# submission2019/cnn-quantization

Measured on NVIDIA H100. Metric: resnet50_w4a4_images_per_s, higher is better.
Workload: dtype f32

## Files before the change

cnn-quantization_b200/csrc/fq_bulk.cuh:

```cuda
#pragma once
#include <cuda_runtime.h>
#include <stdint.h>

#include "fq_device.cuh"

namespace fqb {

constexpr int kConsumers = kThreads;
constexpr int kBulkThreads = kConsumers + 32;
constexpr int kConsumerWarps = kConsumers / 32;
#ifndef FQB_STAGE_VEC
#define FQB_STAGE_VEC 4
#endif
#ifndef FQB_STAGES
#define FQB_STAGES 6
#endif
#ifndef FQB_BULK_CTAS
#define FQB_BULK_CTAS 1
#endif
constexpr int kBulkCtasPerSm = FQB_BULK_CTAS;
constexpr int kStageVec = FQB_STAGE_VEC;
constexpr int kStages = FQB_STAGES;
constexpr unsigned kStageBytes = kStageVec * kConsumers * 16u;
#ifndef FQB_BULK_SPLIT
#define FQB_BULK_SPLIT 1
#endif
constexpr unsigned kBulkSplit = FQB_BULK_SPLIT;

__device__ __forceinline__ void consumer_sync() { cta_sync(); }

__device__ __forceinline__ unsigned smem_u32(const void* p) { return static_cast<unsigned>(__cvta_generic_to_shared(p)); }
__device__ __forceinline__ void mbar_init(unsigned bar, unsigned count) {
  asm volatile("mbarrier.init.shared::cta.b64 [%0], %1;" ::"r"(bar), "r"(count) : "memory");
}
__device__ __forceinline__ void mbar_fence_init() { asm volatile("fence.mbarrier_init.release.cluster;" ::: "memory"); }
__device__ __forceinline__ void mbar_arrive(unsigned bar) {
  asm volatile("{ .reg .b64 st; mbarrier.arrive.shared::cta.b64 st, [%0]; }" ::"r"(bar) : "memory");
}
__device__ __forceinline__ void mbar_arrive_expect_tx(unsigned bar, unsigned bytes) {
  asm volatile("{ .reg .b64 st; mbarrier.arrive.expect_tx.shared::cta.b64 st, [%0], %1; }" ::"r"(bar), "r"(bytes) : "memory");
}
__device__ __forceinline__ bool mbar_try_wait(unsigned bar, unsigned parity) {
  unsigned ok;
  asm volatile(
      "{ .reg .pred p; mbarrier.try_wait.parity.shared::cta.b64 p, [%1], %2; selp.u32 %0, 1, 0, p; }"
      : "=r"(ok)
      : "r"(bar), "r"(parity)
      : "memory");
  return ok != 0;
}
__device__ __forceinline__ void mbar_wait(unsigned bar, unsigned parity) {
  while (!mbar_try_wait(bar, parity)) {
  }
}
__device__ __forceinline__ void bulk_load_one(unsigned dst_smem, const void* src, unsigned bytes, unsigned bar) {
  asm volatile("cp.async.bulk.shared::cluster.global.mbarrier::complete_tx::bytes [%0], [%1], %2, [%3];" ::"r"(dst_smem),
               "l"(src), "r"(bytes), "r"(bar)
               : "memory");
}
__device__ __forceinline__ void bulk_load(unsigned dst_smem, const void* src, unsigned bytes, unsigned bar) {
  if (kBulkSplit == 1u) {
    bulk_load_one(dst_smem, src, bytes, bar);
    return;
  }
  constexpr unsigned piece = kStageBytes / kBulkSplit;
  for (unsigned off = 0; off < bytes; off += piece)
    bulk_load_one(dst_smem + off, static_cast<const unsigned char*>(src) + off, min(piece, bytes - off), bar);
}

struct FlatGeo {
  unsigned total_v;
  unsigned stride;
  unsigned stage_v;
  unsigned n_stages;
  unsigned unit_stages;
  unsigned units;
  unsigned channels;
  unsigned cv;
};

struct StageMeta {
  unsigned start;
  unsigned count;
  unsigned tag;
  unsigned pad;
};

struct BulkRing {
  alignas(8) unsigned long long full[kStages];
  alignas(8) unsigned long long empty[kStages];
  StageMeta meta[kStages];
  unsigned nstages;
};

struct RingPos {
  unsigned slot, parity, n;
  __device__ __forceinline__ void init(unsigned nstages = kStages) {
    slot = 0;
    parity = 0;
    n = nstages;
  }
  __device__ __forceinline__ void next() {
    if (++slot == n) {
      slot = 0;
      parity ^= 1u;
    }
  }
};

__device__ __forceinline__ void ring_init(BulkRing& r, unsigned nstages = kStages) {
  if (threadIdx.x == 0) {
    r.nstages = nstages;
#pragma unroll
    for (int s = 0; s < kStages; ++s) {
      mbar_init(smem_u32(&r.full[s]), 1u);
      mbar_init(smem_u32(&r.empty[s]), kConsumerWarps);
    }
    mbar_fence_init();
  }
  __syncthreads();
}

struct TicketPlan {
  unsigned nstatic;
  unsigned first, step;
  unsigned dyn_base;
};

constexpr unsigned kPairOffset = kStageBytes / 2u;

__device__ __forceinline__ FlatGeo half_geo(const FlatGeo& g) {
  FlatGeo h = g;
  h.stage_v = (kStageVec / 2u) * g.stride;
  h.n_stages = (g.total_v + h.stage_v - 1u) / h.stage_v;
  h.unit_stages = 2u * g.unit_stages;
  return h;
}

template <bool REV, bool PAIR = false>
__device__ __forceinline__ void produce_phase(const FlatGeo& g, const float4* src, unsigned* counter, const TicketPlan tp,
                                              BulkRing& r, unsigned char* stage_base, RingPos& pos,
                                              const float4* src2 = nullptr) {
  const unsigned total = g.units;
  unsigned k = 0;
  auto fetch = [&]() -> unsigned {
    unsigned long long t;
    if (k < tp.nstatic)
      t = tp.first + static_cast<unsigned long long>(k) * tp.step;
    else
      t = static_cast<unsigned long long>(tp.dyn_base) + atomicAdd(counter, 1u);
    ++k;
    return t < total ? static_cast<unsigned>(t) : 0xffffffffu;
  };
  unsigned cur = fetch();
  unsigned nxt = (cur != 0xffffffffu) ? fetch() : 0xffffffffu;
  while (cur != 0xffffffffu) {
    const unsigned nxt2 = (nxt != 0xffffffffu) ? fetch() : 0xffffffffu;
    const unsigned u = REV ? total - 1u - cur : cur;
    const unsigned g0 = u * g.unit_stages;
    const unsigned g1 = min(g0 + g.unit_stages, g.n_stages);
    for (unsigned i = g0; i < g1; ++i) {
      const unsigned st = REV ? g1 - 1u - (i - g0) : i;
      const unsigned start = st * g.stage_v;
      const unsigned count = min(g.stage_v, g.total_v - start);
      mbar_wait(smem_u32(&r.empty[pos.slot]), pos.parity ^ 1u);
      r.meta[pos.slot].start = start;
      r.meta[pos.slot].count = count;
      r.meta[pos.slot].tag = 0u;
      const unsigned bar = smem_u32(&r.full[pos.slot]);
      mbar_arrive_expect_tx(bar, PAIR ? count * 32u : count * 16u);
      bulk_load(smem_u32(stage_base + pos.slot * kStageBytes), src + start, count * 16u, bar);
      if (PAIR) bulk_load(smem_u32(stage_base + pos.slot * kStageBytes + kPairOffset), src2 + start, count * 16u, bar);
      pos.next();
    }
    cur = nxt;
    nxt = nxt2;
  }
  mbar_wait(smem_u32(&r.empty[pos.slot]), pos.parity ^ 1u);
  r.meta[pos.slot].start = 0u;
  r.meta[pos.slot].count = 0u;
  mbar_arrive(smem_u32(&r.full[pos.slot]));
  pos.next();
}

struct RowsGeo {
  unsigned rows, row_v;
  unsigned stages_per_row;
  unsigned units_per_row;
};

__device__ __forceinline__ RowsGeo half_rows(const FlatGeo& h, const RowsGeo& rg) {
  RowsGeo r = rg;
  r.stages_per_row = (rg.row_v + h.stage_v - 1u) / h.stage_v;
  r.units_per_row = (r.stages_per_row + h.unit_stages - 1u) / h.unit_stages;
  return r;
}

template <bool REV, bool PAIR = false>
__device__ __forceinline__ void produce_rows_phase(const FlatGeo& g, const RowsGeo& rg, const float4* src, unsigned* counter,
                                                   const TicketPlan tp, BulkRing& r, unsigned char* stage_base, RingPos& pos,
                                                   const float4* src2 = nullptr) {
  const unsigned total = g.units;
  unsigned k = 0;
  auto fetch = [&]() -> unsigned {
    unsigned long long t;
    if (k < tp.nstatic)
      t = tp.first + static_cast<unsigned long long>(k) * tp.step;
    else
      t = static_cast<unsigned long long>(tp.dyn_base) + atomicAdd(counter, 1u);
    ++k;
    return t < total ? static_cast<unsigned>(t) : 0xffffffffu;
  };
  unsigned cur = fetch();
  unsigned nxt = (cur != 0xffffffffu) ? fetch() : 0xffffffffu;
  while (cur != 0xffffffffu) {
    const unsigned nxt2 = (nxt != 0xffffffffu) ? fetch() : 0xffffffffu;
    const unsigned u = REV ? total - 1u - cur : cur;
    const unsigned row = u / rg.units_per_row;
    const unsigned part = u - row * rg.units_per_row;
    const unsigned s0 = part * g.unit_stages;
    const unsigned s1 = min(s0 + g.unit_stages, rg.stages_per_row);
    for (unsigned i = s0; i < s1; ++i) {
      const unsigned st = REV ? s1 - 1u - (i - s0) : i;
      const unsigned off = st * g.stage_v;
      const unsigned start = row * rg.row_v + off;
      const unsigned count = min(g.stage_v, rg.row_v - off);
      mbar_wait(smem_u32(&r.empty[pos.slot]), pos.parity ^ 1u);
      r.meta[pos.slot].start = start;
      r.meta[pos.slot].count = count;
      r.meta[pos.slot].tag = row | (i + 1u == s1 ? 0x80000000u : 0u);
      const unsigned bar = smem_u32(&r.full[pos.slot]);
      mbar_arrive_expect_tx(bar, PAIR ? count * 32u : count * 16u);
      bulk_load(smem_u32(stage_base + pos.slot * kStageBytes), src + start, count * 16u, bar);
      if (PAIR) bulk_load(smem_u32(stage_base + pos.slot * kStageBytes + kPairOffset), src2 + start, count * 16u, bar);
      pos.next();
    }
    cur = nxt;
    nxt = nxt2;
  }
  mbar_wait(smem_u32(&r.empty[pos.slot]), pos.parity ^ 1u);
  r.meta[pos.slot].start = 0u;
  r.meta[pos.slot].count = 0u;
  r.meta[pos.slot].tag = 0u;
  mbar_arrive(smem_u32(&r.full[pos.slot]));
  pos.next();
}

struct PoolGeo {
  unsigned h, w;
  unsigned wt;
  unsigned tiles_per_row;
  unsigned row_pairs;
  unsigned tiles;
  unsigned unit_tiles, units;
  unsigned ow;
  unsigned kind;
};

constexpr unsigned kPoolTop = 1u, kPoolLeft = 2u;

__device__ __forceinline__ void produce_pool3_phase(const FlatGeo& g, const PoolGeo& pg, const float4* src, unsigned* counter,
                                                    const TicketPlan tp, BulkRing& r, unsigned char* stage_base, RingPos& pos) {
  const unsigned total = pg.units;
  unsigned k = 0;
  auto fetch = [&]() -> unsigned {
    unsigned long long t;
    if (k < tp.nstatic)
      t = tp.first + static_cast<unsigned long long>(k) * tp.step;
    else
      t = static_cast<unsigned long long>(tp.dyn_base) + atomicAdd(counter, 1u);
    ++k;
    return t < total ? static_cast<unsigned>(t) : 0xffffffffu;
  };
  const unsigned row_v = pg.w * g.cv;
  const unsigned region_v = (2u * pg.wt + 1u) * g.cv;
  const unsigned per_img = pg.row_pairs * pg.tiles_per_row;
  unsigned cur = fetch();
  unsigned nxt = (cur != 0xffffffffu) ? fetch() : 0xffffffffu;
  while (cur != 0xffffffffu) {
    const unsigned nxt2 = (nxt != 0xffffffffu) ? fetch() : 0xffffffffu;
    const unsigned t0 = cur * pg.unit_tiles;
    const unsigned t1 = min(t0 + pg.unit_tiles, pg.tiles);
    for (unsigned tile = t0; tile < t1; ++tile) {
      const unsigned n = tile / per_img;
      const unsigned rem = tile - n * per_img;
      const unsigned oh = rem / pg.tiles_per_row;
      const unsigned wi = rem - oh * pg.tiles_per_row;
      const bool top = oh > 0u, left = wi > 0u;
      const unsigned skip = left ? 0u : g.cv;
      const unsigned count = region_v - skip;
      const unsigned mid = (n * pg.h + 2u * oh) * row_v + (2u * wi * pg.wt) * g.cv - (left ? g.cv : 0u);
      const unsigned o = ((n * pg.row_pairs + oh) * pg.ow + wi * pg.wt) * g.cv;
      mbar_wait(smem_u32(&r.empty[pos.slot]), pos.parity ^ 1u);
      r.meta[pos.slot].start = o;
      r.meta[pos.slot].count = count;
      r.meta[pos.slot].tag = (top ? kPoolTop : 0u) | (left ? kPoolLeft : 0u);
      const unsigned bar = smem_u32(&r.full[pos.slot]);
      mbar_arrive_expect_tx(bar, count * 16u * (top ? 3u : 2u));
      const unsigned dst = smem_u32(stage_base + pos.slot * kStageBytes) + skip * 16u;
      if (top) bulk_load(dst, src + mid - row_v, count * 16u, bar);
      bulk_load(dst + region_v * 16u, src + mid, count * 16u, bar);
      bulk_load(dst + 2u * region_v * 16u, src + mid + row_v, count * 16u, bar);
      pos.next();
    }
    cur = nxt;
    nxt = nxt2;
  }
  mbar_wait(smem_u32(&r.empty[pos.slot]), pos.parity ^ 1u);
  r.meta[pos.slot].start = 0u;
  r.meta[pos.slot].count = 0u;
  r.meta[pos.slot].tag = 0u;
  mbar_arrive(smem_u32(&r.full[pos.slot]));
  pos.next();
}

template <typename Acc>
__device__ __forceinline__ void consume_pool3_phase(const FlatGeo& g, const PoolGeo& pg, BulkRing& r, const unsigned char* stage_base,
                                                    RingPos& pos, Acc& acc) {
  const unsigned t = threadIdx.x;
  const bool lane0 = (t & 31u) == 0u;
  const bool mine = t < pg.wt * g.cv;
  const unsigned j = t / g.cv, col = t - j * g.cv;
  const unsigned region = (2u * pg.wt + 1u) * g.cv * 16u;
  const unsigned my = smem_u32(stage_base) + ((2u * j) * g.cv + col) * 16u;
  const unsigned nxt = g.cv * 16u;
  for (;;) {
    mbar_wait(smem_u32(&r.full[pos.slot]), pos.parity);
    const StageMeta m = r.meta[pos.slot];
    if (m.count != 0u && mine) {
      const unsigned addr = my + pos.slot * kStageBytes;
      const bool first = (j != 0u) || (m.tag & kPoolLeft);
      acc.pool_begin();
#pragma unroll
      for (int dy = 0; dy < 3; ++dy) {
        if (dy == 0 && !(m.tag & kPoolTop)) continue;
        const unsigned row = addr + dy * region;
        float4 v;
        if (first) {
          lds_vec(row, v);
          acc.pool_tap(v);
        }
        lds_vec(row + nxt, v);
        acc.pool_tap(v);
        lds_vec(row + 2u * nxt, v);
        acc.pool_tap(v);
      }
      acc.pool_end(m.start + t);
    }
    __syncwarp();
    if (lane0) mbar_arrive(smem_u32(&r.empty[pos.slot]));
    pos.next();
    if (m.count == 0u) break;
  }
}

__device__ __forceinline__ void produce_pool_phase(const FlatGeo& g, const PoolGeo& pg, const float4* src, unsigned* counter,
                                                   const TicketPlan tp, BulkRing& r, unsigned char* stage_base, RingPos& pos) {
  const unsigned total = pg.units;
  unsigned k = 0;
  auto fetch = [&]() -> unsigned {
    unsigned long long t;
    if (k < tp.nstatic)
      t = tp.first + static_cast<unsigned long long>(k) * tp.step;
    else
      t = static_cast<unsigned long long>(tp.dyn_base) + atomicAdd(counter, 1u);
    ++k;
    return t < total ? static_cast<unsigned>(t) : 0xffffffffu;
  };
  const unsigned row_v = pg.w * g.cv;
  const unsigned count = pg.wt * g.cv;
  const unsigned per_img = pg.row_pairs * pg.tiles_per_row;
  unsigned cur = fetch();
  unsigned nxt = (cur != 0xffffffffu) ? fetch() : 0xffffffffu;
  while (cur != 0xffffffffu) {
    const unsigned nxt2 = (nxt != 0xffffffffu) ? fetch() : 0xffffffffu;
    const unsigned t0 = cur * pg.unit_tiles;
    const unsigned t1 = min(t0 + pg.unit_tiles, pg.tiles);
    for (unsigned tile = t0; tile < t1; ++tile) {
      const unsigned n = tile / per_img;
      const unsigned rem = tile - n * per_img;
      const unsigned hp = rem / pg.tiles_per_row;
      const unsigned wi = rem - hp * pg.tiles_per_row;
      const unsigned a = (n * pg.h + 2u * hp) * row_v + wi * count;
      const unsigned o = ((n * pg.row_pairs + hp) * pg.ow + wi * (pg.wt / 2u)) * g.cv;
      mbar_wait(smem_u32(&r.empty[pos.slot]), pos.parity ^ 1u);
      r.meta[pos.slot].start = o;
      r.meta[pos.slot].count = count;
      r.meta[pos.slot].tag = 0u;
      const unsigned bar = smem_u32(&r.full[pos.slot]);
      mbar_arrive_expect_tx(bar, count * 32u);
      bulk_load(smem_u32(stage_base + pos.slot * kStageBytes), src + a, count * 16u, bar);
      bulk_load(smem_u32(stage_base + pos.slot * kStageBytes + kPairOffset), src + a + row_v, count * 16u, bar);
      pos.next();
    }
    cur = nxt;
    nxt = nxt2;
  }
  mbar_wait(smem_u32(&r.empty[pos.slot]), pos.parity ^ 1u);
  r.meta[pos.slot].start = 0u;
  r.meta[pos.slot].count = 0u;
  r.meta[pos.slot].tag = 0u;
  mbar_arrive(smem_u32(&r.full[pos.slot]));
  pos.next();
}

template <typename Acc>
__device__ __forceinline__ void consume_pool_phase(const FlatGeo& g, const PoolGeo& pg, BulkRing& r, const unsigned char* stage_base,
                                                   RingPos& pos, Acc& acc) {
  const unsigned t = threadIdx.x;
  const bool lane0 = (t & 31u) == 0u;
  const bool mine = t < (pg.wt / 2u) * g.cv;
  const unsigned j = t / g.cv, col = t - j * g.cv;
  const unsigned my = smem_u32(stage_base) + ((2u * j) * g.cv + col) * 16u;
  const unsigned nxt = g.cv * 16u;
  for (;;) {
    mbar_wait(smem_u32(&r.full[pos.slot]), pos.parity);
    const StageMeta m = r.meta[pos.slot];
    if (m.count != 0u && mine) {
      const unsigned addr = my + pos.slot * kStageBytes;
      float4 a0, a1, b0, b1;
      lds_vec(addr, a0);
      lds_vec(addr + nxt, a1);
      lds_vec(addr + kPairOffset, b0);
      lds_vec(addr + kPairOffset + nxt, b1);
      acc.pooled(a0, a1, b0, b1, m.start + t);
    }
    __syncwarp();
    if (lane0) mbar_arrive(smem_u32(&r.empty[pos.slot]));
    pos.next();
    if (m.count == 0u) break;
  }
}

template <typename Acc>
__device__ __forceinline__ void consume_phase(const FlatGeo& g, BulkRing& r, const unsigned char* stage_base, RingPos& pos,
                                              Acc& acc) {
  const unsigned t = threadIdx.x;
  const bool lane0 = (t & 31u) == 0u;
  const unsigned my = smem_u32(stage_base) + t * 16u;
  const unsigned step = g.stride * 16u;
  for (;;) {
    mbar_wait(smem_u32(&r.full[pos.slot]), pos.parity);
    const StageMeta m = r.meta[pos.slot];
    const unsigned addr = my + pos.slot * kStageBytes;
    if (m.count == g.stage_v) {
      if (t < g.stride) {
        float4 x[kStageVec];
#pragma unroll
        for (int i = 0; i < kStageVec; ++i) lds_vec(addr + i * step, x[i]);
#pragma unroll
        for (int i = 0; i < kStageVec; ++i) acc.consume(x[i], m.start + t + i * g.stride);
      }
    } else if (m.count != 0u) {
#pragma unroll
      for (int i = 0; i < kStageVec; ++i) {
        const unsigned idx = t + i * g.stride;
        if (t < g.stride && idx < m.count) {
          float4 x;
          lds_vec(addr + i * step, x);
          acc.consume(x, m.start + idx);
        }
      }
    }
    acc.stage_end(m);
    __syncwarp();
    if (lane0) mbar_arrive(smem_u32(&r.empty[pos.slot]));
    pos.next();
    if (m.count == 0u) break;
  }
}

template <typename Acc>
__device__ __forceinline__ void consume_pair_phase(const FlatGeo& g, BulkRing& r, const unsigned char* stage_base, RingPos& pos,
                                                   Acc& acc) {
  static_assert(kStageVec % 2u == 0u, "a pair stage is split in two halves");
  constexpr int kHalf = kStageVec / 2;
  const unsigned t = threadIdx.x;
  const bool lane0 = (t & 31u) == 0u;
  const unsigned my = smem_u32(stage_base) + t * 16u;
  const unsigned step = g.stride * 16u;
  for (;;) {
    mbar_wait(smem_u32(&r.full[pos.slot]), pos.parity);
    const StageMeta m = r.meta[pos.slot];
    const unsigned addr = my + pos.slot * kStageBytes;
    if (m.count == g.stage_v) {
      if (t < g.stride) {
        float4 x[kHalf], y[kHalf];
#pragma unroll
        for (int i = 0; i < kHalf; ++i) {
          lds_vec(addr + i * step, x[i]);
          lds_vec(addr + kPairOffset + i * step, y[i]);
        }
#pragma unroll
        for (int i = 0; i < kHalf; ++i) acc.consume2(x[i], y[i], m.start + t + i * g.stride);
      }
    } else if (m.count != 0u) {
#pragma unroll
      for (int i = 0; i < kHalf; ++i) {
        const unsigned idx = t + i * g.stride;
        if (t < g.stride && idx < m.count) {
          float4 x, y;
          lds_vec(addr + i * step, x);
          lds_vec(addr + kPairOffset + i * step, y);
          acc.consume2(x, y, m.start + idx);
        }
      }
    }
    acc.stage_end(m);
    __syncwarp();
    if (lane0) mbar_arrive(smem_u32(&r.empty[pos.slot]));
    pos.next();
    if (m.count == 0u) break;
  }
}

}
```

cnn-quantization_b200/csrc/fq_cl.cuh:

```cuda
#pragma once

namespace fqb {

__device__ __forceinline__ unsigned enc_ordered(float x) {
  const unsigned b = __float_as_uint(x);
  return (b & 0x80000000u) ? ~b : (b | 0x80000000u);
}
__device__ __forceinline__ float dec_ordered(unsigned e) {
  return __uint_as_float((e & 0x80000000u) ? (e & 0x7fffffffu) : ~e);
}

constexpr unsigned kAccU = 2u * kMaxNhwcChannels;
constexpr unsigned kAccD = 3u * kMaxNhwcChannels;

struct ClView {
  unsigned* amin_inv;
  unsigned* amax;
  double* asum;
  double* asq;
  double* aabs;
};
__device__ __forceinline__ ClView cl_view(const FusedArgs& A, unsigned bank) {
  ClView v;
  v.amin_inv = A.amin_inv + bank * kAccU;
// ... 482 lines not shown
__device__ __noinline__ LeafParam cl_channel_param(const FusedArgs& A, const ClView& acc, unsigned rep, unsigned C, unsigned c,
                                                   float mu, double n, bool alloc, bool do_export) {
  auto umax = [](unsigned a, unsigned b) { return a > b ? a : b; };
  const unsigned lo = cl_rep_reduce(acc.amin_inv, rep, C, c, 0u, umax);
  const unsigned hi = cl_rep_reduce(acc.amax, rep, C, c, 0u, umax);
  const double sa = DEV ? cl_rep_reduce(acc.aabs, rep, C, c, 0.0, OpAdd()) : 0.0;
  const float cb = A.bias ? __ldg(A.bias + c) : 0.f;
  const float mn = __fadd_rn(dec_ordered(~lo), cb), mx = __fadd_rn(dec_ordered(hi), cb);
  const float b = DEV ? static_cast<float>(sa / n) : 0.f;
  const bool need_sd = A.range_mode == FQB200_RANGE_GAUS || A.range_mode == FQB200_RANGE_KSTD || do_export;
  const float sd = need_sd ? cl_std(acc, rep, C, c, n) : 0.f;
  const float aux = alloc ? ld_ws(A.gbits + c) : static_cast<float>(A.num_bits);
  LeafParam q;
  if constexpr (LEAF == FQB200_LEAF_MIDTREAD) {
    float rng;
    q = mid_tread_param(A, aux, mn, mx, mu, b, rng);
    if (do_export) export_stats(A, c, mn, mx, mu, b, sd, rng, 0.f, aux, q);
  } else {
    float delta, offset;
    solve_range(A, mn, mx, mu, b, sd, aux, delta, offset);
    q = make_leaf_param(LEAF, delta, offset, aux);
    if (do_export) export_stats(A, c, mn, mx, mu, b, sd, delta, offset, aux, q);
  }
  return q;
}

struct ClCtx {
  const FlatGeo* g;
  BulkRing* ring;
  unsigned char* stages;
  unsigned char* cbuf;
  RingPos pos;
  ClView acc;
  unsigned rep_base, c0;
  bool active;
};

__device__ __noinline__ void cl_phase_s1(const FusedArgs& A, ClCtx& cx, float (&kshift)[4]) {
  const FlatGeo& g = *cx.g;
  ClStats1 s1;
  s1.init(A, cx.c0, cx.active);
#pragma unroll
  for (int i = 0; i < 4; ++i) kshift[i] = s1.k[i];
  RingPos pos = cx.pos;
  consume_phase(g, *cx.ring, cx.stages, pos, s1);
  cx.pos = pos;
  s1.flush();
  if (blockIdx.x == 0) stamp(A, 13);
  unsigned umn[4], umx[4];
#pragma unroll
  for (int i = 0; i < 4; ++i) {
    umn[i] = ~enc_ordered(s1.mn[i]);
    umx[i] = enc_ordered(s1.mx[i]);
  }
  const ClView& acc = cx.acc;
  const unsigned rb = cx.rep_base;
  cl_combine_s1(cx.cbuf, g.cv, g.stride, umn, umx, s1.s, s1.q, acc.amin_inv + rb, acc.amax + rb, acc.asum + rb, acc.asq + rb);
}

__device__ __noinline__ void cl_phase_s2(const FusedArgs& A, ClCtx& cx, const float (&mean)[4]) {
  const FlatGeo& g = *cx.g;
  ClStats2 s2;
  s2.init(A, cx.c0, cx.active, mean);
  RingPos pos = cx.pos;
  consume_phase(g, *cx.ring, cx.stages, pos, s2);
  cx.pos = pos;
  s2.flush();
  if (blockIdx.x == 0) stamp(A, 14);
  const ClView& acc = cx.acc;
  const unsigned rb = cx.rep_base;
  cl_combine_add_f64(cx.cbuf, g.cv, g.stride, s2.sa, acc.aabs + rb, s2.sa, nullptr, s2.sa, nullptr);
}

template <int LEAF, bool HIST>
__device__ __noinline__ void cl_phase_apply(const FusedArgs& A, ClCtx& cx, const LeafParam (&lp)[4], unsigned* hist) {
  const FlatGeo& g = *cx.g;
  const unsigned t = threadIdx.x;
  if (HIST) {
    for (unsigned i = t; i < kHistWords; i += kConsumers) hist[i] = 0u;
    consumer_sync();
  }
  ClApply<LEAF, HIST> ap{A, hist};
  ap.init(cx.c0, cx.active, lp);
  RingPos pos = cx.pos;
  if (A.pool.tiles) {
    if (A.pool.kind == 3u)
      consume_pool3_phase(g, A.pool, *cx.ring, cx.stages, pos, ap);
    else
      consume_pool_phase(g, A.pool, *cx.ring, cx.stages, pos, ap);
  } else if (A.residual) {
    const FlatGeo h = half_geo(g);
    consume_pair_phase(h, *cx.ring, cx.stages, pos, ap);
  } else {
    consume_phase(g, *cx.ring, cx.stages, pos, ap);
  }
  cx.pos = pos;
  if (HIST) {
    consumer_sync();
    const unsigned bins = static_cast<unsigned>(A.hist_bins);
    const unsigned copies = max(1u, min(static_cast<unsigned>(kWarps), kHistWords / bins));
    for (unsigned b = t; b < bins; b += kConsumers) {
      unsigned long long cnt = 0;
      for (unsigned w = 0; w < copies; ++w) cnt += hist[w * bins + b];
      if (cnt) atomicAdd(A.hist + b, cnt);
    }
    if (LEAF == FQB200_LEAF_MIDTREAD && A.hist_clamped && cx.active) {
#pragma unroll
      for (int i = 0; i < 4; ++i) {
        if (ap.nlo[i]) atomicAdd(A.hist_clamped + 2u * (cx.c0 + i), static_cast<unsigned long long>(ap.nlo[i]));
        if (ap.nhi[i]) atomicAdd(A.hist_clamped + 2u * (cx.c0 + i) + 1u, static_cast<unsigned long long>(ap.nhi[i]));
      }
    }
  }
}

constexpr unsigned kClStagingBytes = 4u * kConsumers * 8u;
constexpr unsigned kClTableChannels = 1024;
constexpr unsigned kClCombineBytes = kClStagingBytes + kClTableChannels * 4u;

template <int LEAF, bool DEV, bool HIST>
__global__ void __launch_bounds__(kBulkThreads, kBulkCtasPerSm) fq_cl_kernel(const __grid_constant__ FusedArgs A) {
  extern __shared__ __align__(128) unsigned char fq_dyn[];
  unsigned char* stages = fq_dyn;
  unsigned char* cbuf = fq_dyn + kStages * kStageBytes;
  float* tab_mean = reinterpret_cast<float*>(cbuf + kClStagingBytes);
  unsigned* hist = reinterpret_cast<unsigned*>(stages + (kStages - 1) * kStageBytes);
  __shared__ BulkRing ring;
  __shared__ LeaderSmem lsm;
  __shared__ alignas(8) unsigned long long solver_done;
  const FlatGeo& g = A.flat;
  const unsigned C = g.channels, cv = g.cv;
  const unsigned launch = ld_ws(&A.sync->launch_count);
  const unsigned bank = launch & 1u;
  const unsigned tag = launch + 1u;
  const bool alloc = (LEAF == FQB200_LEAF_MIDTREAD) || (A.bit_alloc && A.num_bits <= 4);
  const bool aux_needs_b = alloc && LEAF != FQB200_LEAF_MIDTREAD && A.prior == FQB200_PRIOR_B;
  const bool solver_in_s2 = alloc && !aux_needs_b && DEV && gridDim.x > 1u;
  __shared__ alignas(8) unsigned long long phase_go[2];
  if (threadIdx.x == 0) {
    mbar_init(smem_u32(&solver_done), 1u);
    mbar_init(smem_u32(&phase_go[0]), 1u);
    mbar_init(smem_u32(&phase_go[1]), 1u);
  }
  const unsigned nstages = HIST ? kStages - 1u : kStages;
  ring_init(ring, nstages);

  if (threadIdx.x >= kConsumers) {
    if (threadIdx.x == kConsumers) {
      RingPos pos;
      pos.init(nstages);
      const float4* src = reinterpret_cast<const float4*>(A.in);
      const TicketPlan all = {2u, blockIdx.x, gridDim.x, 2u * gridDim.x};
      const TicketPlan no0 = {blockIdx.x == 0 ? 0u : 2u, blockIdx.x - 1u, gridDim.x - 1u, 2u * (gridDim.x - 1u)};
      produce_phase<false>(g, src, &A.sync->unit_counter[0], all, ring, stages, pos);
      if (DEV) {
        mbar_wait(smem_u32(&phase_go[0]), 0u);
        if (solver_in_s2 && blockIdx.x == 0) mbar_wait(smem_u32(&solver_done), 0u);
        produce_phase<true>(g, src, &A.sync->unit_counter[1], solver_in_s2 ? no0 : all, ring, stages, pos);
      }
      if (!A.stats_only) {
        mbar_wait(smem_u32(&phase_go[1]), 0u);
        if (A.pool.tiles && A.pool.kind == 3u)
          produce_pool3_phase(g, A.pool, src, &A.sync->unit_counter[2], all, ring, stages, pos);
        else if (A.pool.tiles)
          produce_pool_phase(g, A.pool, src, &A.sync->unit_counter[2], all, ring, stages, pos);
        else if (A.residual)
          produce_phase<!DEV, true>(half_geo(g), src, &A.sync->unit_counter[2], all, ring, stages, pos,
                                    reinterpret_cast<const float4*>(A.residual));
        else
          produce_phase<!DEV>(g, src, &A.sync->unit_counter[2], all, ring, stages, pos);
      }
    }
    return;
  }

  const unsigned t = threadIdx.x;
  const bool active = t < g.stride;
  const bool direct = cv == g.stride;
  const unsigned col = active ? t % cv : 0u;
  const unsigned c0 = 4u * col;
  const double n = A.n_per_group;
  const ClView acc = cl_view(A, bank);
  const unsigned rep = A.nhwc_rep;
  const unsigned rep_base = (blockIdx.x % rep) * C;
  unsigned epoch = 0;
  if (blockIdx.x == 0) stamp(A, 0);

  if (blockIdx.x == gridDim.x - 1u) {
    const ClView other = cl_view(A, bank ^ 1u);
    uint4* zu = reinterpret_cast<uint4*>(other.amin_inv);
    uint4* zd = reinterpret_cast<uint4*>(other.asum);
    const uint4 z = make_uint4(0u, 0u, 0u, 0u);
    for (unsigned i = t; i < kAccU / 4u; i += kConsumers) zu[i] = z;
    for (unsigned i = t; i < kAccD / 2u; i += kConsumers) zd[i] = z;
  }

  ClCtx cx;
  cx.g = &g;
  cx.ring = &ring;
  cx.stages = stages;
  cx.cbuf = cbuf;
  cx.pos.init(nstages);
  cx.acc = acc;
  cx.rep_base = rep_base;
  cx.c0 = c0;
  cx.active = active;
  float kshift[4];
  cl_phase_s1(A, cx, kshift);
  if (t == 0) mbar_arrive(smem_u32(&phase_go[DEV ? 0 : 1]));
  if (blockIdx.x == 0) stamp(A, 1);
  grid_barrier_cl(A.sync, epoch);
  if (blockIdx.x == 0) stamp(A, 4);

  float mean[4];
  if (direct) {
#pragma unroll
    for (int i = 0; i < 4; ++i)
      mean[i] = static_cast<float>(cl_mean(acc, rep, C, c0 + i, kshift[i], (A.bias && active) ? __ldg(A.bias + c0 + i) : 0.f, n));
  } else {
    for (unsigned c = t; c < C; c += kConsumers)
      tab_mean[c] = static_cast<float>(cl_mean(acc, rep, C, c, ld_tensor(A.in + c), A.bias ? __ldg(A.bias + c) : 0.f, n));
    consumer_sync();
#pragma unroll
    for (int i = 0; i < 4; ++i) mean[i] = tab_mean[c0 + i];
  }

  if (alloc && !aux_needs_b && blockIdx.x == 0) {
    cl_solve_aux(A, acc, lsm, tag, false, !solver_in_s2);
    stamp(A, 12);
    if (t == 0) mbar_arrive(smem_u32(&solver_done));
  }

  if constexpr (DEV) {
    cl_phase_s2(A, cx, mean);
    if (t == 0) mbar_arrive(smem_u32(&phase_go[1]));
    if (blockIdx.x == 0) stamp(A, 5);
    grid_barrier_cl(A.sync, epoch);
    if (blockIdx.x == 0) stamp(A, 8);
    if (aux_needs_b && blockIdx.x == 0) cl_solve_aux(A, acc, lsm, tag, true, true);
  }
  if (alloc && !solver_in_s2) {
    if (t == 0)
      while (ld_acquire_u32(&A.sync->aux_ready) != tag) __nanosleep(40);
    consumer_sync();
  }

  LeafParam lp[4];
  const bool do_export = A.out_stats != nullptr && blockIdx.x == 0;
  if (direct) {
#pragma unroll
    for (int i = 0; i < 4; ++i) lp[i] = cl_channel_param<LEAF, DEV>(A, acc, rep, C, c0 + i, mean[i], n, alloc, do_export && active);
  } else {
    LeafParam* tab_lp = reinterpret_cast<LeafParam*>(cbuf);
    consumer_sync();
    for (unsigned c = t; c < C; c += kConsumers) tab_lp[c] = cl_channel_param<LEAF, DEV>(A, acc, rep, C, c, tab_mean[c], n, alloc, do_export);
    consumer_sync();
#pragma unroll
    for (int i = 0; i < 4; ++i) lp[i] = tab_lp[c0 + i];
  }
  if (blockIdx.x == 0) stamp(A, 7);

  if (!A.stats_only) {
    cl_phase_apply<LEAF, HIST>(A, cx, lp, hist);
    if (blockIdx.x == 0) stamp(A, 9);
  }
  grid_exit_cl(A.sync);
}

template <bool GRID>
struct ClGiven {
  const FusedArgs& A;
  LeafParam q[4];
  float r[4], bias[4];
  bool fast;
  template <bool FAST>
  __device__ __forceinline__ void one(const float4& v, unsigned off) {
    const float x[4] = {v.x, v.y, v.z, v.w};
    float y[4], gq[4];
#pragma unroll
    for (int i = 0; i < 4; ++i) {
      Divisor dv;
      dv.s = q[i].a;
      dv.r = r[i];
      dv.fast = FAST;
      y[i] = leaf_apply<FQB200_LEAF_TORCH, FAST>(__fadd_rn(x[i], bias[i]), q[i], dv, 0.f, gq[i]);
    }
    st_tensor(reinterpret_cast<float4*>(A.out) + off, make_float4(y[0], y[1], y[2], y[3]));
    if (GRID) st_tensor(reinterpret_cast<float4*>(A.grid_out) + off, make_float4(gq[0], gq[1], gq[2], gq[3]));
  }
  __device__ __forceinline__ void consume(const float4& v, unsigned off) {
    if (fast)
      one<true>(v, off);
    else
      one<false>(v, off);
  }
  __device__ __forceinline__ void stage_end(const StageMeta&) {}
};

template <bool GRID>
__global__ void __launch_bounds__(kBulkThreads, kBulkCtasPerSm) fq_cl_given_kernel(const __grid_constant__ FusedArgs A) {
  extern __shared__ __align__(128) unsigned char fq_dyn[];
  __shared__ BulkRing ring;
  const FlatGeo& g = A.flat;
  ring_init(ring);
  if (threadIdx.x >= kConsumers) {
    if (threadIdx.x == kConsumers) {
      RingPos pos;
      pos.init();
      const TicketPlan tp = {0xffffffffu, blockIdx.x, gridDim.x, 0u};
      produce_phase<false>(g, reinterpret_cast<const float4*>(A.in), nullptr, tp, ring, fq_dyn, pos);
    }
    return;
  }
  const unsigned t = threadIdx.x;
  const bool active = t < g.stride;
  const unsigned c0 = active ? 4u * (t % g.cv) : 0u;
  ClGiven<GRID> ap{A};
  ap.fast = true;
#pragma unroll
  for (int i = 0; i < 4; ++i) {
    const unsigned c = c0 + i;
    const unsigned pi = A.given_per_group ? c : 0u;
    const float bits = A.g_bits ? __ldg(A.g_bits + c) : static_cast<float>(A.num_bits);
    ap.q[i] = make_leaf_param(FQB200_LEAF_TORCH, __ldg(A.g_delta + pi), __ldg(A.g_offset + pi), bits);
    const Divisor dv = make_divisor(ap.q[i].a);
    ap.r[i] = dv.r;
    ap.fast = ap.fast && dv.fast;
    ap.bias[i] = (A.bias && active) ? __ldg(A.bias + c) : 0.f;
  }
  RingPos pos;
  pos.init();
  consume_phase(g, ring, fq_dyn, pos, ap);
}

__global__ void __launch_bounds__(kBulkThreads, kBulkCtasPerSm) fq_cl_given_fused_kernel(const __grid_constant__ FusedArgs A) {
  extern __shared__ __align__(128) unsigned char fq_dyn[];
  __shared__ BulkRing ring;
  const FlatGeo& g = A.flat;
  ring_init(ring);
  if (threadIdx.x >= kConsumers) {
    if (threadIdx.x == kConsumers) {
      RingPos pos;
      pos.init();
      const float4* src = reinterpret_cast<const float4*>(A.in);
      const TicketPlan tp = {0xffffffffu, blockIdx.x, gridDim.x, 0u};
      if (A.pool.tiles && A.pool.kind == 3u)
        produce_pool3_phase(g, A.pool, src, nullptr, tp, ring, fq_dyn, pos);
      else if (A.pool.tiles)
        produce_pool_phase(g, A.pool, src, nullptr, tp, ring, fq_dyn, pos);
      else if (A.residual)
        produce_phase<false, true>(half_geo(g), src, nullptr, tp, ring, fq_dyn, pos, reinterpret_cast<const float4*>(A.residual));
      else
        produce_phase<false>(g, src, nullptr, tp, ring, fq_dyn, pos);
    }
    return;
  }
  const unsigned t = threadIdx.x;
  const bool active = t < g.stride;
  const unsigned c0 = active ? 4u * (t % g.cv) : 0u;
  LeafParam lp[4];
#pragma unroll
  for (int i = 0; i < 4; ++i) {
    const unsigned c = c0 + i;
    const float bits = A.g_bits ? __ldg(A.g_bits + c) : static_cast<float>(A.num_bits);
    lp[i] = make_leaf_param(FQB200_LEAF_TORCH, __ldg(A.g_delta + c), __ldg(A.g_offset + c), bits);
  }
  ClApply<FQB200_LEAF_TORCH, false> ap{A, nullptr};
  ap.init(c0, active, lp);
  RingPos pos;
  pos.init();
  if (A.pool.tiles && A.pool.kind == 3u)
    consume_pool3_phase(g, A.pool, ring, fq_dyn, pos, ap);
  else if (A.pool.tiles)
    consume_pool_phase(g, A.pool, ring, fq_dyn, pos, ap);
  else if (A.residual)
    consume_pair_phase(half_geo(g), ring, fq_dyn, pos, ap);
  else
    consume_phase(g, ring, fq_dyn, pos, ap);
}

struct LeafBulkArgs {
  FlatGeo flat;
  const float* in;
  float* out;
  const float* noise;
  LeafParam q;
};

template <bool NOISE>
struct LeafBulk {
  const LeafBulkArgs& A;
  Divisor dv;
  template <bool FAST>
  __device__ __forceinline__ void one(const float4& v, const float4& nz, unsigned off) {
    float gq;
    float4 y;
    y.x = leaf_apply<FQB200_LEAF_COMPILED, FAST, NOISE>(v.x, A.q, dv, NOISE ? nz.x : 0.f, gq);
    y.y = leaf_apply<FQB200_LEAF_COMPILED, FAST, NOISE>(v.y, A.q, dv, NOISE ? nz.y : 0.f, gq);
    y.z = leaf_apply<FQB200_LEAF_COMPILED, FAST, NOISE>(v.z, A.q, dv, NOISE ? nz.z : 0.f, gq);
    y.w = leaf_apply<FQB200_LEAF_COMPILED, FAST, NOISE>(v.w, A.q, dv, NOISE ? nz.w : 0.f, gq);
    st_tensor(reinterpret_cast<float4*>(A.out) + off, y);
  }
  __device__ __forceinline__ void consume(const float4& v, unsigned off) {
    if (dv.fast)
      one<true>(v, v, off);
    else
      one<false>(v, v, off);
  }
  __device__ __forceinline__ void consume2(const float4& v, const float4& nz, unsigned off) {
    if (dv.fast)
      one<true>(v, nz, off);
    else
      one<false>(v, nz, off);
  }
  __device__ __forceinline__ void stage_end(const StageMeta&) {}
};

template <bool NOISE>
__global__ void __launch_bounds__(kBulkThreads, kBulkCtasPerSm) fq_leaf_bulk_kernel(const __grid_constant__ LeafBulkArgs A) {
  extern __shared__ __align__(128) unsigned char fq_dyn[];
  __shared__ BulkRing ring;
  const FlatGeo g = NOISE ? half_geo(A.flat) : A.flat;
  ring_init(ring);
  if (threadIdx.x >= kConsumers) {
    if (threadIdx.x == kConsumers) {
      RingPos pos;
      pos.init();
      const TicketPlan tp = {0xffffffffu, blockIdx.x, gridDim.x, 0u};
      produce_phase<false, NOISE>(g, reinterpret_cast<const float4*>(A.in), nullptr, tp, ring, fq_dyn, pos,
                                  reinterpret_cast<const float4*>(A.noise));
    }
    return;
  }
  LeafBulk<NOISE> ap{A, make_divisor(A.q.a)};
  RingPos pos;
  pos.init();
  if (NOISE)
    consume_pair_phase(g, ring, fq_dyn, pos, ap);
  else
    consume_phase(g, ring, fq_dyn, pos, ap);
}

struct ClBca1 {
  const FusedArgs& A;
  LeafParam q[4];
  float r[4], bias[4], fr[4], fy[4];
  double sr[4], sy[4];
  unsigned cnt[4], n;
  bool fast;
  __device__ __forceinline__ void flush() {
#pragma unroll
    for (int i = 0; i < 4; ++i) {
      sr[i] += static_cast<double>(fr[i]);
      sy[i] += static_cast<double>(fy[i]);
      fr[i] = 0.f;
      fy[i] = 0.f;
    }
    n = 0;
  }
  template <bool FAST>
  __device__ __forceinline__ void one(const float4& v) {
    const float x[4] = {v.x, v.y, v.z, v.w};
#pragma unroll
    for (int i = 0; i < 4; ++i) {
      Divisor dv;
      dv.s = q[i].a;
      dv.r = r[i];
      dv.fast = FAST;
      float gq;
      const float xb = __fadd_rn(x[i], bias[i]);
      const float y = leaf_apply<FQB200_LEAF_TORCH, FAST>(xb, q[i], dv, 0.f, gq);
      const float rr = (A.relu_passthrough && xb < 0.f) ? 0.f : xb;
      fr[i] = __fadd_rn(fr[i], rr);
      fy[i] = __fadd_rn(fy[i], y);
      cnt[i] += rr > 0.f ? 1u : 0u;
    }
  }
  __device__ __forceinline__ void consume(const float4& v, unsigned) {
    if (fast)
      one<true>(v);
    else
      one<false>(v);
  }
  __device__ __forceinline__ void stage_end(const StageMeta&) {
    if (++n == kClChunkStages) flush();
  }
};

struct ClBca2 {
  const FusedArgs& A;
  LeafParam q[4];
  float r[4], bias[4], qb[4];
  bool fast;
  template <bool FAST>
  __device__ __forceinline__ void one(const float4& v, unsigned off) {
    const float x[4] = {v.x, v.y, v.z, v.w};
    float y[4];
#pragma unroll
    for (int i = 0; i < 4; ++i) {
      Divisor dv;
      dv.s = q[i].a;
      dv.r = r[i];
// ... 122 lines not shown
    if (!(m.tag & 0x80000000u)) return;
    const float a = warp_reduce(mn, OpMin()), b = warp_reduce(mx, OpMax());
    const unsigned w = threadIdx.x >> 5, l = threadIdx.x & 31u;
    consumer_sync();
    if (l == 0) {
      scratch[w] = a;
      scratch[kWarps + w] = b;
    }
    consumer_sync();
    if (w == 0) {
      float c = (l < kWarps) ? scratch[l] : INFINITY, d = (l < kWarps) ? scratch[kWarps + l] : -INFINITY;
#pragma unroll
      for (int o = kWarps / 2; o > 0; o >>= 1) {
        c = fminf(c, __shfl_xor_sync(0xffffffffu, c, o));
        d = fmaxf(d, __shfl_xor_sync(0xffffffffu, d, o));
      }
      if (l == 0) {
        const unsigned row = m.tag & 0x7fffffffu;
        red_max_u32(acc.amin_inv + row, ~enc_ordered(c));
        red_max_u32(acc.amax + row, enc_ordered(d));
      }
    }
    mn = INFINITY;
    mx = -INFINITY;
  }
};

struct RowsApply {
  const FusedArgs& A;
  LeafParam q;
  Divisor dv;
  float bias[4];
  LeafParam rq;
  Divisor rdv;
  float rbias[4];
  bool rquant;
  __device__ __forceinline__ void init_residual(unsigned c0, bool active) {
    rquant = A.residual != nullptr && A.residual_stats != nullptr;
    rq.a = 1.f;
    rq.b = 0.f;
    rq.c = 0.f;
    rq.flags = 0;
#pragma unroll
    for (int i = 0; i < 4; ++i) rbias[i] = 0.f;
    if (rquant) {
      rq.a = __ldg(A.residual_stats + 8);
      rq.b = __ldg(A.residual_stats + 9);
      rq.c = __ldg(A.residual_stats + 10);
      rq.flags = static_cast<int>(__ldg(A.residual_stats + 11));
      if (A.residual_bias && active) {
#pragma unroll
        for (int i = 0; i < 4; ++i) rbias[i] = __ldg(A.residual_bias + c0 + i);
      }
    }
    rdv = make_divisor(rq.a);
    if (rquant && !rdv.fast) dv.fast = false;
    rdv.fast = dv.fast;
  }
  template <bool FAST, bool PAIR>
  __device__ __forceinline__ void one(const float4& v, const float4& r0, unsigned off) {
    float gq;
    float4 y;
    float4 r = r0;
    if (PAIR && rquant) {
      r.x = leaf_apply<FQB200_LEAF_COMPILED, FAST>(__fadd_rn(r0.x, rbias[0]), rq, rdv, 0.f, gq);
      r.y = leaf_apply<FQB200_LEAF_COMPILED, FAST>(__fadd_rn(r0.y, rbias[1]), rq, rdv, 0.f, gq);
      r.z = leaf_apply<FQB200_LEAF_COMPILED, FAST>(__fadd_rn(r0.z, rbias[2]), rq, rdv, 0.f, gq);
      r.w = leaf_apply<FQB200_LEAF_COMPILED, FAST>(__fadd_rn(r0.w, rbias[3]), rq, rdv, 0.f, gq);
    }
    y.x = leaf_apply<FQB200_LEAF_COMPILED, FAST>(__fadd_rn(v.x, bias[0]), q, dv, 0.f, gq);
    y.y = leaf_apply<FQB200_LEAF_COMPILED, FAST>(__fadd_rn(v.y, bias[1]), q, dv, 0.f, gq);
    y.z = leaf_apply<FQB200_LEAF_COMPILED, FAST>(__fadd_rn(v.z, bias[2]), q, dv, 0.f, gq);
    y.w = leaf_apply<FQB200_LEAF_COMPILED, FAST>(__fadd_rn(v.w, bias[3]), q, dv, 0.f, gq);
    if (PAIR) {
      y.x = __fadd_rn(y.x, r.x);
      y.y = __fadd_rn(y.y, r.y);
      y.z = __fadd_rn(y.z, r.z);
      y.w = __fadd_rn(y.w, r.w);
      if (A.residual_relu) {
        y.x = y.x < 0.f ? 0.f : y.x;
        y.y = y.y < 0.f ? 0.f : y.y;
        y.z = y.z < 0.f ? 0.f : y.z;
        y.w = y.w < 0.f ? 0.f : y.w;
      }
    }
    st_tensor(reinterpret_cast<float4*>(A.out) + off, y);
  }
  __device__ __forceinline__ void consume(const float4& v, unsigned off) {
    if (dv.fast)
      one<true, false>(v, v, off);
    else
      one<false, false>(v, v, off);
  }
  __device__ __forceinline__ void consume2(const float4& v, const float4& r, unsigned off) {
    if (dv.fast)
      one<true, true>(v, r, off);
    else
      one<false, true>(v, r, off);
  }
  __device__ __forceinline__ void stage_end(const StageMeta&) {}
  float pm[4];
  __device__ __forceinline__ void pool_begin() {
#pragma unroll
    for (int i = 0; i < 4; ++i) pm[i] = -INFINITY;
  }
  __device__ __forceinline__ void pool_tap(const float4& v) {
    auto mx = [](float p, float q) { return (q > p || q != q) ? q : p; };
    pm[0] = mx(pm[0], v.x);
    pm[1] = mx(pm[1], v.y);
    pm[2] = mx(pm[2], v.z);
    pm[3] = mx(pm[3], v.w);
  }
  __device__ __forceinline__ void pool_end(unsigned off) {
    float gq;
    float4 y;
    if (dv.fast) {
      y.x = leaf_apply<FQB200_LEAF_COMPILED, true>(__fadd_rn(pm[0], bias[0]), q, dv, 0.f, gq);
      y.y = leaf_apply<FQB200_LEAF_COMPILED, true>(__fadd_rn(pm[1], bias[1]), q, dv, 0.f, gq);
      y.z = leaf_apply<FQB200_LEAF_COMPILED, true>(__fadd_rn(pm[2], bias[2]), q, dv, 0.f, gq);
      y.w = leaf_apply<FQB200_LEAF_COMPILED, true>(__fadd_rn(pm[3], bias[3]), q, dv, 0.f, gq);
    } else {
      y.x = leaf_apply<FQB200_LEAF_COMPILED, false>(__fadd_rn(pm[0], bias[0]), q, dv, 0.f, gq);
      y.y = leaf_apply<FQB200_LEAF_COMPILED, false>(__fadd_rn(pm[1], bias[1]), q, dv, 0.f, gq);
      y.z = leaf_apply<FQB200_LEAF_COMPILED, false>(__fadd_rn(pm[2], bias[2]), q, dv, 0.f, gq);
      y.w = leaf_apply<FQB200_LEAF_COMPILED, false>(__fadd_rn(pm[3], bias[3]), q, dv, 0.f, gq);
    }
    st_tensor(reinterpret_cast<float4*>(A.pool_out) + off, y);
  }
  __device__ __forceinline__ void pooled(const float4& a0, const float4& a1, const float4& b0, const float4& b1, unsigned off) {
    pool_begin();
    pool_tap(a0);
    pool_tap(a1);
    pool_tap(b0);
    pool_tap(b1);
    pool_end(off);
  }
};

__global__ void __launch_bounds__(kBulkThreads, kBulkCtasPerSm) fq_rows_kernel(const __grid_constant__ FusedArgs A) {
  extern __shared__ __align__(128) unsigned char fq_dyn[];
  __shared__ BulkRing ring;
  __shared__ LeaderSmem lsm;
  __shared__ float scratch[2 * kWarps];
  const FlatGeo& g = A.flat;
  const RowsGeo& rg = A.rows;
  const unsigned bank = ld_ws(&A.sync->launch_count) & 1u;
  ring_init(ring);
  if (threadIdx.x >= kConsumers) {
    if (threadIdx.x == kConsumers) {
      RingPos pos;
      pos.init();
      const float4* src = reinterpret_cast<const float4*>(A.in);
      const TicketPlan all = {2u, blockIdx.x, gridDim.x, 2u * gridDim.x};
      produce_rows_phase<false>(g, rg, src, &A.sync->unit_counter[0], all, ring, fq_dyn, pos);
      if (!A.stats_only) {
        if (A.pool.tiles && A.pool.kind == 3u) {
          produce_pool3_phase(g, A.pool, src, &A.sync->unit_counter[2], all, ring, fq_dyn, pos);
        } else if (A.pool.tiles) {
          produce_pool_phase(g, A.pool, src, &A.sync->unit_counter[2], all, ring, fq_dyn, pos);
        } else if (A.residual) {
          const FlatGeo h = half_geo(g);
          produce_rows_phase<true, true>(h, half_rows(h, rg), src, &A.sync->unit_counter[2], all, ring, fq_dyn, pos,
                                         reinterpret_cast<const float4*>(A.residual));
        } else {
          produce_rows_phase<true>(g, rg, src, &A.sync->unit_counter[2], all, ring, fq_dyn, pos);
        }
      }
    }
    return;
  }
  const unsigned t = threadIdx.x;
  const bool active = t < g.stride;
  const unsigned c0 = active ? 4u * (t % g.cv) : 0u;
  const ClView acc = cl_view(A, bank);
  unsigned epoch = 0;
  RingPos pos;
  pos.init();
  if (blockIdx.x == 0) stamp(A, 0);
  if (blockIdx.x == gridDim.x - 1u) {
    const ClView other = cl_view(A, bank ^ 1u);
    uint4* zu = reinterpret_cast<uint4*>(other.amin_inv);
    uint4* zd = reinterpret_cast<uint4*>(other.asum);
    const uint4 z = make_uint4(0u, 0u, 0u, 0u);
    for (unsigned i = t; i < kAccU / 4u; i += kConsumers) zu[i] = z;
    for (unsigned i = t; i < kAccD / 2u; i += kConsumers) zd[i] = z;
  }
  float bias[4];
#pragma unroll
  for (int i = 0; i < 4; ++i) bias[i] = (A.bias && active) ? __ldg(A.bias + c0 + i) : 0.f;
  {
    RowsStats s1{A, scratch, acc, {bias[0], bias[1], bias[2], bias[3]}, INFINITY, -INFINITY};
    consume_phase(g, ring, fq_dyn, pos, s1);
  }
  if (blockIdx.x == 0) stamp(A, 1);
  grid_barrier_cl(A.sync, epoch);
  if (blockIdx.x == 0) stamp(A, 4);
  const unsigned R = rg.rows;
  float mn, mx;
  if (A.scope == FQB200_SCOPE_GROUP_MEAN) {
    double smin = 0.0, smax = 0.0;
    for (unsigned r = t; r < R; r += kConsumers) {
      smin += static_cast<double>(dec_ordered(~ld_ws(acc.amin_inv + r)));
      smax += static_cast<double>(dec_ordered(ld_ws(acc.amax + r)));
    }
    smin = block_reduce(smin, OpAdd(), lsm.d);
    smax = block_reduce(smax, OpAdd(), lsm.d);
    mn = static_cast<float>(smin / R);
    mx = static_cast<float>(smax / R);
  } else {
    float lmin = INFINITY, lmax = -INFINITY;
    for (unsigned r = t; r < R; r += kConsumers) {
      lmin = fminf(lmin, dec_ordered(~ld_ws(acc.amin_inv + r)));
      lmax = fmaxf(lmax, dec_ordered(ld_ws(acc.amax + r)));
    }
    mn = block_reduce(lmin, OpMin(), lsm.f);
    mx = block_reduce(lmax, OpMax(), lsm.f);
  }
  float delta, offset;
  solve_range(A, mn, mx, 0.f, 0.f, 0.f, static_cast<float>(A.num_bits), delta, offset);
  const LeafParam q = make_leaf_param(FQB200_LEAF_COMPILED, delta, offset, static_cast<float>(A.num_bits), A.relu_passthrough != 0);
  if (blockIdx.x == 0 && t == 0) export_stats(A, 0, mn, mx, 0.f, 0.f, 0.f, delta, offset, static_cast<float>(A.num_bits), q);
  if (blockIdx.x == 0) stamp(A, 7);
  if (!A.stats_only) {
    RowsApply ap{A, q, make_divisor(q.a), {bias[0], bias[1], bias[2], bias[3]}};
    ap.init_residual(c0, active);
    if (A.pool.tiles && A.pool.kind == 3u)
      consume_pool3_phase(g, A.pool, ring, fq_dyn, pos, ap);
    else if (A.pool.tiles)
      consume_pool_phase(g, A.pool, ring, fq_dyn, pos, ap);
    else if (A.residual)
      consume_pair_phase(half_geo(g), ring, fq_dyn, pos, ap);
    else
      consume_phase(g, ring, fq_dyn, pos, ap);
    if (blockIdx.x == 0) stamp(A, 9);
  }
  grid_exit_cl(A.sync);
}

}
```

Measured before the change: 9063.

## Split flat phases into fine-grained tail units and flip phase traversal directions

produce_phase now carves the last few stages per CTA into single-stage work units, so dynamic ticket scheduling can balance the tail of each phase across CTAs more finely. Pool producers gain a REV template parameter, and the multi-phase kernels flip traversal directions: the stats phase runs reversed and later phases run forward (or reversed when DEV). The aim is to improve L2 reuse between consecutive passes over the same tensor and to cut straggler imbalance at phase ends. The cost is more atomic ticket fetches for the tail units and a possible loss of locality if the new ordering does not match what stays in cache.

```diff
diff --git a/cnn-quantization_b200/csrc/fq_bulk.cuh b/cnn-quantization_b200/csrc/fq_bulk.cuh
--- a/cnn-quantization_b200/csrc/fq_bulk.cuh
+++ b/cnn-quantization_b200/csrc/fq_bulk.cuh
@@ -137,11 +137,16 @@
   return h;
 }
 
+constexpr unsigned kTailStagesPerCta = 4;
+
 template <bool REV, bool PAIR = false>
 __device__ __forceinline__ void produce_phase(const FlatGeo& g, const float4* src, unsigned* counter, const TicketPlan tp,
                                               BulkRing& r, unsigned char* stage_base, RingPos& pos,
                                               const float4* src2 = nullptr) {
-  const unsigned total = g.units;
+  const unsigned tail = min(g.n_stages, kTailStagesPerCta * gridDim.x);
+  const unsigned body = g.n_stages - tail;
+  const unsigned nbody = (body + g.unit_stages - 1u) / g.unit_stages;
+  const unsigned total = nbody + tail;
   unsigned k = 0;
   auto fetch = [&]() -> unsigned {
     unsigned long long t;
@@ -156,9 +161,19 @@
   unsigned nxt = (cur != 0xffffffffu) ? fetch() : 0xffffffffu;
   while (cur != 0xffffffffu) {
     const unsigned nxt2 = (nxt != 0xffffffffu) ? fetch() : 0xffffffffu;
-    const unsigned u = REV ? total - 1u - cur : cur;
-    const unsigned g0 = u * g.unit_stages;
-    const unsigned g1 = min(g0 + g.unit_stages, g.n_stages);
+    unsigned g0, g1;
+    if (cur < nbody) {
+      g0 = cur * g.unit_stages;
+      g1 = min(g0 + g.unit_stages, body);
+    } else {
+      g0 = body + (cur - nbody);
+      g1 = g0 + 1u;
+    }
+    if (REV) {
+      const unsigned m0 = g.n_stages - g1;
+      g1 = g.n_stages - g0;
+      g0 = m0;
+    }
     for (unsigned i = g0; i < g1; ++i) {
       const unsigned st = REV ? g1 - 1u - (i - g0) : i;
       const unsigned start = st * g.stage_v;
@@ -259,6 +274,7 @@
 
 constexpr unsigned kPoolTop = 1u, kPoolLeft = 2u;
 
+template <bool REV>
 __device__ __forceinline__ void produce_pool3_phase(const FlatGeo& g, const PoolGeo& pg, const float4* src, unsigned* counter,
                                                     const TicketPlan tp, BulkRing& r, unsigned char* stage_base, RingPos& pos) {
   const unsigned total = pg.units;
@@ -279,9 +295,11 @@
   unsigned nxt = (cur != 0xffffffffu) ? fetch() : 0xffffffffu;
   while (cur != 0xffffffffu) {
     const unsigned nxt2 = (nxt != 0xffffffffu) ? fetch() : 0xffffffffu;
-    const unsigned t0 = cur * pg.unit_tiles;
+    const unsigned u = REV ? total - 1u - cur : cur;
+    const unsigned t0 = u * pg.unit_tiles;
     const unsigned t1 = min(t0 + pg.unit_tiles, pg.tiles);
-    for (unsigned tile = t0; tile < t1; ++tile) {
+    for (unsigned i = t0; i < t1; ++i) {
+      const unsigned tile = REV ? t1 - 1u - (i - t0) : i;
       const unsigned n = tile / per_img;
       const unsigned rem = tile - n * per_img;
       const unsigned oh = rem / pg.tiles_per_row;
@@ -354,6 +372,7 @@
   }
 }
 
+template <bool REV>
 __device__ __forceinline__ void produce_pool_phase(const FlatGeo& g, const PoolGeo& pg, const float4* src, unsigned* counter,
                                                    const TicketPlan tp, BulkRing& r, unsigned char* stage_base, RingPos& pos) {
   const unsigned total = pg.units;
@@ -374,9 +393,11 @@
   unsigned nxt = (cur != 0xffffffffu) ? fetch() : 0xffffffffu;
   while (cur != 0xffffffffu) {
     const unsigned nxt2 = (nxt != 0xffffffffu) ? fetch() : 0xffffffffu;
-    const unsigned t0 = cur * pg.unit_tiles;
+    const unsigned u = REV ? total - 1u - cur : cur;
+    const unsigned t0 = u * pg.unit_tiles;
     const unsigned t1 = min(t0 + pg.unit_tiles, pg.tiles);
-    for (unsigned tile = t0; tile < t1; ++tile) {
+    for (unsigned i = t0; i < t1; ++i) {
+      const unsigned tile = REV ? t1 - 1u - (i - t0) : i;
       const unsigned n = tile / per_img;
       const unsigned rem = tile - n * per_img;
       const unsigned hp = rem / pg.tiles_per_row;
diff --git a/cnn-quantization_b200/csrc/fq_cl.cuh b/cnn-quantization_b200/csrc/fq_cl.cuh
--- a/cnn-quantization_b200/csrc/fq_cl.cuh
+++ b/cnn-quantization_b200/csrc/fq_cl.cuh
@@ -658,23 +658,23 @@
       const float4* src = reinterpret_cast<const float4*>(A.in);
       const TicketPlan all = {2u, blockIdx.x, gridDim.x, 2u * gridDim.x};
       const TicketPlan no0 = {blockIdx.x == 0 ? 0u : 2u, blockIdx.x - 1u, gridDim.x - 1u, 2u * (gridDim.x - 1u)};
-      produce_phase<false>(g, src, &A.sync->unit_counter[0], all, ring, stages, pos);
+      produce_phase<true>(g, src, &A.sync->unit_counter[0], all, ring, stages, pos);
       if (DEV) {
         mbar_wait(smem_u32(&phase_go[0]), 0u);
         if (solver_in_s2 && blockIdx.x == 0) mbar_wait(smem_u32(&solver_done), 0u);
-        produce_phase<true>(g, src, &A.sync->unit_counter[1], solver_in_s2 ? no0 : all, ring, stages, pos);
+        produce_phase<false>(g, src, &A.sync->unit_counter[1], solver_in_s2 ? no0 : all, ring, stages, pos);
       }
       if (!A.stats_only) {
         mbar_wait(smem_u32(&phase_go[1]), 0u);
         if (A.pool.tiles && A.pool.kind == 3u)
-          produce_pool3_phase(g, A.pool, src, &A.sync->unit_counter[2], all, ring, stages, pos);
+          produce_pool3_phase<DEV>(g, A.pool, src, &A.sync->unit_counter[2], all, ring, stages, pos);
         else if (A.pool.tiles)
-          produce_pool_phase(g, A.pool, src, &A.sync->unit_counter[2], all, ring, stages, pos);
+          produce_pool_phase<DEV>(g, A.pool, src, &A.sync->unit_counter[2], all, ring, stages, pos);
         else if (A.residual)
-          produce_phase<!DEV, true>(half_geo(g), src, &A.sync->unit_counter[2], all, ring, stages, pos,
-                                    reinterpret_cast<const float4*>(A.residual));
+          produce_phase<DEV, true>(half_geo(g), src, &A.sync->unit_counter[2], all, ring, stages, pos,
+                                   reinterpret_cast<const float4*>(A.residual));
         else
-          produce_phase<!DEV>(g, src, &A.sync->unit_counter[2], all, ring, stages, pos);
+          produce_phase<DEV>(g, src, &A.sync->unit_counter[2], all, ring, stages, pos);
       }
     }
     return;
@@ -851,9 +851,9 @@
       const float4* src = reinterpret_cast<const float4*>(A.in);
       const TicketPlan tp = {0xffffffffu, blockIdx.x, gridDim.x, 0u};
       if (A.pool.tiles && A.pool.kind == 3u)
-        produce_pool3_phase(g, A.pool, src, nullptr, tp, ring, fq_dyn, pos);
+        produce_pool3_phase<false>(g, A.pool, src, nullptr, tp, ring, fq_dyn, pos);
       else if (A.pool.tiles)
-        produce_pool_phase(g, A.pool, src, nullptr, tp, ring, fq_dyn, pos);
+        produce_pool_phase<false>(g, A.pool, src, nullptr, tp, ring, fq_dyn, pos);
       else if (A.residual)
         produce_phase<false, true>(half_geo(g), src, nullptr, tp, ring, fq_dyn, pos, reinterpret_cast<const float4*>(A.residual));
       else
@@ -1282,18 +1282,18 @@
       pos.init();
       const float4* src = reinterpret_cast<const float4*>(A.in);
       const TicketPlan all = {2u, blockIdx.x, gridDim.x, 2u * gridDim.x};
-      produce_rows_phase<false>(g, rg, src, &A.sync->unit_counter[0], all, ring, fq_dyn, pos);
+      produce_rows_phase<true>(g, rg, src, &A.sync->unit_counter[0], all, ring, fq_dyn, pos);
       if (!A.stats_only) {
         if (A.pool.tiles && A.pool.kind == 3u) {
-          produce_pool3_phase(g, A.pool, src, &A.sync->unit_counter[2], all, ring, fq_dyn, pos);
+          produce_pool3_phase<false>(g, A.pool, src, &A.sync->unit_counter[2], all, ring, fq_dyn, pos);
         } else if (A.pool.tiles) {
-          produce_pool_phase(g, A.pool, src, &A.sync->unit_counter[2], all, ring, fq_dyn, pos);
+          produce_pool_phase<false>(g, A.pool, src, &A.sync->unit_counter[2], all, ring, fq_dyn, pos);
         } else if (A.residual) {
           const FlatGeo h = half_geo(g);
-          produce_rows_phase<true, true>(h, half_rows(h, rg), src, &A.sync->unit_counter[2], all, ring, fq_dyn, pos,
-                                         reinterpret_cast<const float4*>(A.residual));
+          produce_rows_phase<false, true>(h, half_rows(h, rg), src, &A.sync->unit_counter[2], all, ring, fq_dyn, pos,
+                                          reinterpret_cast<const float4*>(A.residual));
         } else {
-          produce_rows_phase<true>(g, rg, src, &A.sync->unit_counter[2], all, ring, fq_dyn, pos);
+          produce_rows_phase<false>(g, rg, src, &A.sync->unit_counter[2], all, ring, fq_dyn, pos);
         }
       }
     }
```

Result: no change. 9093, median of 6 (+0.3%).
